# injun-baek/Video-Depth-Normal-v2

Measured on AMD Instinct MI355X. Metric: depth frames/sec at 518x518, ViT-L, higher is better.
Workload: dtype f16x3; 1 GPU; DepthAnythingV2(vitl) batch=8 518x518 streams/GPU, memory bank full (S=6); replicas per GPU; lanes=2, precision=f16x3, ranks=1, backend=none, attention_pv_products=1

## Files before the change

video-depth-normal-v2_amd/csrc/spatial.hip:

```cpp
#include "common.hpp"
#include <stddef.h>

namespace {

__device__ __forceinline__ void ac_coord(int o, float scale, int in, int& i0, int& i1, float& l1) {
#pragma clang fp contract(off)
  const float src = scale * (float)o;
  i0 = (int)src;
  i0 = i0 < in - 1 ? i0 : in - 1;
  i1 = i0 < in - 1 ? i0 + 1 : i0;
  l1 = src - (float)i0;
}

template <int DT>
__global__ __launch_bounds__(256) void upsample_kernel(const typename Half<DT>::T* __restrict__ x,
                                                       const typename Half<DT>::T* __restrict__ xl,
                                                       typename Half<DT>::T* __restrict__ y,
                                                       typename Half<DT>::T* __restrict__ yl, int B, int IH, int IW,
                                                       int OH, int OW, int C) {
  using T = typename Half<DT>::T;
  using V8 = typename Half<DT>::V8;
  const int cv = C >> 3;
  const size_t total = (size_t)B * OH * OW * cv;
  const float sy = OH > 1 ? (float)(IH - 1) / (float)(OH - 1) : 0.f;
  const float sx = OW > 1 ? (float)(IW - 1) / (float)(OW - 1) : 0.f;
  for (size_t i = blockIdx.x * (size_t)256 + threadIdx.x; i < total; i += (size_t)gridDim.x * 256) {
    const int c8 = (int)(i % cv);
    size_t pix = i / cv;
    const int ox = (int)(pix % OW);
    pix /= OW;
    const int oy = (int)(pix % OH);
    const int b = (int)(pix / OH);
    int y0, y1, x0, x1;
    float ly, lx;
    ac_coord(oy, sy, IH, y0, y1, ly);
    ac_coord(ox, sx, IW, x0, x1, lx);
    const size_t xo = (size_t)b * IH * IW * C + c8 * 8;
    const size_t o00 = xo + ((size_t)y0 * IW + x0) * C, o01 = xo + ((size_t)y0 * IW + x1) * C;
    const size_t o10 = xo + ((size_t)y1 * IW + x0) * C, o11 = xo + ((size_t)y1 * IW + x1) * C;
    const V8 v00 = *(const V8*)(x + o00), v01 = *(const V8*)(x + o01);
    const V8 v10 = *(const V8*)(x + o10), v11 = *(const V8*)(x + o11);
    V8 l00, l01, l10, l11, o, ol;
    if (xl) {
      l00 = *(const V8*)(xl + o00); l01 = *(const V8*)(xl + o01);
      l10 = *(const V8*)(xl + o10); l11 = *(const V8*)(xl + o11);
    }
#pragma unroll
    for (int e = 0; e < 8; ++e) {
      float a00 = (float)v00[e], a01 = (float)v01[e], a10 = (float)v10[e], a11 = (float)v11[e];
      if (xl) { a00 += (float)l00[e]; a01 += (float)l01[e]; a10 += (float)l10[e]; a11 += (float)l11[e]; }
      const float top = (1.f - lx) * a00 + lx * a01;
      const float bot = (1.f - lx) * a10 + lx * a11;
      const float r = (1.f - ly) * top + ly * bot;
      if (yl) { T a, b2; split_rtz(r, a, b2); o[e] = a; ol[e] = b2; }
      else o[e] = (T)r;
    }
    *(V8*)(y + i * 8) = o;
    if (yl) *(V8*)(yl + i * 8) = ol;
  }
}

__global__ __launch_bounds__(256) void upsample_f32_kernel(const float* __restrict__ x, float* __restrict__ y, int B,
                                                           int IH, int IW, int OH, int OW, int relu) {
  const size_t total = (size_t)B * OH * OW;
  const float sy = OH > 1 ? (float)(IH - 1) / (float)(OH - 1) : 0.f;
  const float sx = OW > 1 ? (float)(IW - 1) / (float)(OW - 1) : 0.f;
  for (size_t i = blockIdx.x * (size_t)256 + threadIdx.x; i < total; i += (size_t)gridDim.x * 256) {
    const int ox = (int)(i % OW);
    const size_t t = i / OW;
    const int oy = (int)(t % OH);
    const int b = (int)(t / OH);
    int y0, y1, x0, x1;
    float ly, lx;
    ac_coord(oy, sy, IH, y0, y1, ly);
    ac_coord(ox, sx, IW, x0, x1, lx);
    const float* xb = x + (size_t)b * IH * IW;
    const float top = (1.f - lx) * xb[y0 * IW + x0] + lx * xb[y0 * IW + x1];
    const float bot = (1.f - lx) * xb[y1 * IW + x0] + lx * xb[y1 * IW + x1];
    float v = (1.f - ly) * top + ly * bot;
    if (relu) v = fmaxf(v, 0.f);
    y[i] = v;
  }
}

template <int DT>
__global__ __launch_bounds__(256) void patchify_kernel(const float* __restrict__ img,
                                                       typename Half<DT>::T* __restrict__ rows,
                                                       typename Half<DT>::T* __restrict__ rows_lo, int B, int H, int W,
                                                       int ldk) {
  using T = typename Half<DT>::T;
  using V8 = typename Half<DT>::V8;
  const int ph = H / 14, pw = W / 14;
  const int kv = ldk >> 3;
  const size_t total = (size_t)B * ph * pw * kv;
  for (size_t i = blockIdx.x * (size_t)256 + threadIdx.x; i < total; i += (size_t)gridDim.x * 256) {
    const int k8 = (int)(i % kv);
    size_t row = i / kv;
    const int px = (int)(row % pw);
    const size_t t = row / pw;
    const int py = (int)(t % ph);
    const int b = (int)(t / ph);
    V8 o, ol;
#pragma unroll
    for (int e = 0; e < 8; ++e) {
      const int k = k8 * 8 + e;
      float v = 0.f;
      if (k < 588) {
        const int c = k / 196, rem = k - c * 196;
        const int ky = rem / 14, kx = rem - ky * 14;
        v = img[(((size_t)b * 3 + c) * H + py * 14 + ky) * W + px * 14 + kx];
      }
      if (rows_lo) { T a, b2; split_rtz(v, a, b2); o[e] = a; ol[e] = b2; }
      else o[e] = (T)v;
    }
    *(V8*)(rows + i * 8) = o;
    if (rows_lo) *(V8*)(rows_lo + i * 8) = ol;
  }
}

__global__ void fill_row_kernel(float* __restrict__ x, const float* __restrict__ vec, int B, int rows_per_b, int row,
                                int C) {
  const int i = blockIdx.x * blockDim.x + threadIdx.x;
  if (i >= B * C) return;
  const int b = i / C, c = i - b * C;
  x[((size_t)b * rows_per_b + row) * C + c] = vec[c];
}

__device__ __forceinline__ void cubic_w(float t, float w[4]) {
  const float A = -0.75f;
  const float x0 = t + 1.f, x1 = t, x2 = 1.f - t, x3 = 2.f - t;
  w[0] = ((A * x0 - 5.f * A) * x0 + 8.f * A) * x0 - 4.f * A;
  w[1] = ((A + 2.f) * x1 - (A + 3.f)) * x1 * x1 + 1.f;
  w[2] = ((A + 2.f) * x2 - (A + 3.f)) * x2 * x2 + 1.f;
  w[3] = ((A * x3 - 5.f * A) * x3 + 8.f * A) * x3 - 4.f * A;
}

__global__ void bicubic_kernel(const float* __restrict__ src, float* __restrict__ dst, int ih, int iw, int oh, int ow,
                               int C, float inv_sy, float inv_sx) {
  const size_t total = (size_t)oh * ow * C;
  for (size_t i = blockIdx.x * (size_t)blockDim.x + threadIdx.x; i < total; i += (size_t)gridDim.x * blockDim.x) {
    const int c = (int)(i % C);
    const size_t p = i / C;
    const int ox = (int)(p % ow), oy = (int)(p / ow);
    const float fy = ((float)oy + 0.5f) * inv_sy - 0.5f;
    const float fx = ((float)ox + 0.5f) * inv_sx - 0.5f;
    const int iy = (int)floorf(fy), ix = (int)floorf(fx);
    float wy[4], wx[4];
    cubic_w(fy - (float)iy, wy);
    cubic_w(fx - (float)ix, wx);
    float acc = 0.f;
#pragma unroll
    for (int a = 0; a < 4; ++a) {
      int yy = iy - 1 + a;
      yy = yy < 0 ? 0 : (yy > ih - 1 ? ih - 1 : yy);
      float rowv = 0.f;
#pragma unroll
      for (int bq = 0; bq < 4; ++bq) {
        int xx = ix - 1 + bq;
        xx = xx < 0 ? 0 : (xx > iw - 1 ? iw - 1 : xx);
        rowv += wx[bq] * src[((size_t)yy * iw + xx) * C + c];
      }
      acc += wy[a] * rowv;
    }
    dst[i] = acc;
  }
}

__device__ __forceinline__ void halfpixel_coord(int o, int in, int out, int& i, float& t) {
  const long long den = 2ll * out, num = (2ll * o + 1) * in - out;
  long long q = num / den, r = num - q * den;
  if (r < 0) { r += den; --q; }
  i = (int)q;
  t = (float)r / (float)den;
}

struct PrepNorm { float mean[3], inv_std[3]; };
__global__ __launch_bounds__(256) void preprocess_kernel(const uint8_t* __restrict__ src, float* __restrict__ dst, int n, int ih, int iw,
                                                         int oh, int ow, int swap_rb, PrepNorm nm) {
  const size_t per = (size_t)oh * ow, total = per * n;
  for (size_t i = blockIdx.x * (size_t)256 + threadIdx.x; i < total; i += (size_t)gridDim.x * 256) {
    const int f = (int)(i / per);
    const size_t p = i - (size_t)f * per;
    const int ox = (int)(p % ow), oy = (int)(p / ow);
    int iy, ix;
    float ty, tx;
    halfpixel_coord(oy, ih, oh, iy, ty);
    halfpixel_coord(ox, iw, ow, ix, tx);
    float wy[4], wx[4];
    cubic_w(ty, wy);
    cubic_w(tx, wx);
    const uint8_t* img = src + (size_t)f * ih * iw * 3;
    float acc[3] = {0.f, 0.f, 0.f};
#pragma unroll
    for (int a = 0; a < 4; ++a) {
      int yy = iy - 1 + a;
      yy = yy < 0 ? 0 : (yy > ih - 1 ? ih - 1 : yy);
      float rowv[3] = {0.f, 0.f, 0.f};
#pragma unroll
      for (int bq = 0; bq < 4; ++bq) {
        int xx = ix - 1 + bq;
        xx = xx < 0 ? 0 : (xx > iw - 1 ? iw - 1 : xx);
        const uint8_t* px = img + ((size_t)yy * iw + xx) * 3;
#pragma unroll
        for (int c = 0; c < 3; ++c) rowv[c] += wx[bq] * ((float)px[c] / 255.0f);
      }
#pragma unroll
      for (int c = 0; c < 3; ++c) acc[c] += wy[a] * rowv[c];
    }
#pragma unroll
    for (int c = 0; c < 3; ++c) {
      const int sc = swap_rb ? 2 - c : c;
      dst[((size_t)f * 3 + c) * per + p] = (acc[sc] - nm.mean[c]) * nm.inv_std[c];
    }
  }
}

template <int DT>
__global__ __launch_bounds__(256) void head_out_kernel(const typename Half<DT>::T* __restrict__ feat,
                                                       const typename Half<DT>::T* __restrict__ feat_lo,
                                                       const float* __restrict__ w, float bias,
                                                       float* __restrict__ depth, int M, int C, int relu) {
  using V8 = typename Half<DT>::V8;
  __shared__ float sw[64];
  if (threadIdx.x < C) sw[threadIdx.x] = w[threadIdx.x];
  __syncthreads();
  for (size_t m = blockIdx.x * (size_t)256 + threadIdx.x; m < (size_t)M; m += (size_t)gridDim.x * 256) {
    float acc = bias;
    for (int c = 0; c < C; c += 8) {
      const V8 v = *(const V8*)(feat + m * C + c);
#pragma unroll
      for (int e = 0; e < 8; ++e) acc += sw[c + e] * (float)v[e];
      if (feat_lo) {
        const V8 vl = *(const V8*)(feat_lo + m * C + c);
#pragma unroll
        for (int e = 0; e < 8; ++e) acc += sw[c + e] * (float)vl[e];
      }
    }
    depth[m] = relu ? fmaxf(acc, 0.f) : acc;
  }
}

__global__ __launch_bounds__(256) void mask_down1_kernel(const float* __restrict__ depth, float* __restrict__ out,
                                                         int B, int H, int W, int OH, int OW,
                                                         const float* __restrict__ w) {
  __shared__ float sw[53];
  if (threadIdx.x < 53) sw[threadIdx.x] = w[threadIdx.x];
  __syncthreads();
  const size_t total = (size_t)B * OH * OW;
  for (size_t i = blockIdx.x * (size_t)256 + threadIdx.x; i < total; i += (size_t)gridDim.x * 256) {
    const int ox = (int)(i % OW);
    const size_t t = i / OW;
    const int oy = (int)(t % OH);
    const int b = (int)(t / OH);
    float in[9];
#pragma unroll
    for (int ky = 0; ky < 3; ++ky)
#pragma unroll
      for (int kx = 0; kx < 3; ++kx) {
        const int iy = oy * 2 - 1 + ky, ix = ox * 2 - 1 + kx;
        float v = 0.f;
        if (iy >= 0 && iy < H && ix >= 0 && ix < W) v = 1.f / (1.f + expf(-depth[((size_t)b * H + iy) * W + ix]));
        in[ky * 3 + kx] = v;
      }
    float ch[4], mean = 0.f;
#pragma unroll
    for (int c = 0; c < 4; ++c) {
      float a = sw[36 + c];
#pragma unroll
      for (int k = 0; k < 9; ++k) a += sw[c * 9 + k] * in[k];
      ch[c] = a;
      mean += a;
    }
    mean *= 0.25f;
    float var = 0.f;
#pragma unroll
    for (int c = 0; c < 4; ++c) var += (ch[c] - mean) * (ch[c] - mean);
    const float rstd = 1.f / sqrtf(var * 0.25f + 1e-6f);
    float o = sw[52];
#pragma unroll
    for (int c = 0; c < 4; ++c) o += sw[48 + c] * gelu_erf((ch[c] - mean) * rstd * sw[40 + c] + sw[44 + c]);
    out[i] = o;
  }
}

__global__ __launch_bounds__(128) void mask_down2_kernel(const float* __restrict__ in, float* __restrict__ out, int B,
                                                         int H, int W, int OH, int OW, const float* __restrict__ w) {
  __shared__ float sw[2598];
  for (int i = threadIdx.x; i < 2598; i += 128) sw[i] = w[i];
  __syncthreads();
  const size_t i = blockIdx.x * (size_t)128 + threadIdx.x;
  if (i >= (size_t)B * OH * OW) return;
  const int ox = (int)(i % OW);
  const size_t t = i / OW;
  const int oy = (int)(t % OH);
  const int b = (int)(t / OH);
  float px[49];
#pragma unroll
  for (int ky = 0; ky < 7; ++ky)
#pragma unroll
    for (int kx = 0; kx < 7; ++kx) px[ky * 7 + kx] = in[((size_t)b * H + oy * 7 + ky) * W + ox * 7 + kx];
  float ch[49], mean = 0.f;
#pragma unroll
  for (int c = 0; c < 49; ++c) {
    float a = sw[2401 + c];
#pragma unroll
    for (int k = 0; k < 49; ++k) a += sw[c * 49 + k] * px[k];
    ch[c] = a;
    mean += a;
  }
  mean *= (1.f / 49.f);
  float var = 0.f;
#pragma unroll
  for (int c = 0; c < 49; ++c) var += (ch[c] - mean) * (ch[c] - mean);
  const float rstd = 1.f / sqrtf(var * (1.f / 49.f) + 1e-6f);
  float o = sw[2597];
#pragma unroll
  for (int c = 0; c < 49; ++c)
    o += sw[2548 + c] * gelu_erf((ch[c] - mean) * rstd * sw[2450 + c] + sw[2499 + c]);
  out[i] = o;
}

constexpr int DW_TH = 8, DW_CB = 32, DW_PS = 36;
__global__ __launch_bounds__(256) void dwconv7_kernel(const float* __restrict__ x, float* __restrict__ y, int B, int H,
                                                      int W, int C, const float* __restrict__ w,
                                                      const float* __restrict__ bias, int WT) {
  extern __shared__ __attribute__((aligned(16))) char smem[];
  float* sw = (float*)smem;
  float* sx = sw + 49 * DW_CB;
  const int cblocks = C / DW_CB, rtiles = (H + DW_TH - 1) / DW_TH, ctiles = (W + WT - 1) / WT;
  int bid = blockIdx.x;
  const int cb = (bid % cblocks) * DW_CB;
  bid /= cblocks;
  const int x0 = (bid % ctiles) * WT;
  bid /= ctiles;
  const int oy0 = (bid % rtiles) * DW_TH, b = bid / rtiles;
  const int Wt = (W - x0) < WT ? (W - x0) : WT;
  const int WP = WT + 6;
  for (int i = threadIdx.x; i < 49 * (DW_CB / 4); i += 256) {
    const int t = i / (DW_CB / 4), v = i - t * (DW_CB / 4);
    *(f32x4*)(sw + t * DW_CB + v * 4) = *(const f32x4*)(w + (size_t)t * C + cb + v * 4);
  }
  for (int i = threadIdx.x; i < (DW_TH + 6) * WP * (DW_CB / 4); i += 256) {
    const int v = i % (DW_CB / 4);
    const int p = i / (DW_CB / 4);
    const int r = p / WP, cx = p - r * WP;
    const int iy = oy0 - 3 + r, ix = x0 + cx - 3;
    f32x4 val = {0.f, 0.f, 0.f, 0.f};
    if (iy >= 0 && iy < H && ix >= 0 && ix < W) val = *(const f32x4*)(x + (((size_t)b * H + iy) * W + ix) * C + cb + v * 4);
    *(f32x4*)(sx + (size_t)(r * WP + cx) * DW_PS + v * 4) = val;
  }
  __syncthreads();
  const int v = threadIdx.x & 7, pl = threadIdx.x >> 3;
  const int runs_per_row = (Wt + 3) / 4;
  const f32x4 bv = *(const f32x4*)(bias + cb + v * 4);
  for (int run = pl; run < DW_TH * runs_per_row; run += 32) {
    const int ry = run / runs_per_row, ox0 = (run - ry * runs_per_row) * 4;
    if (oy0 + ry >= H) break;
    f32x4 acc[4] = {bv, bv, bv, bv};
#pragma unroll
    for (int ky = 0; ky < 7; ++ky) {
      const float* row = sx + (size_t)((ry + ky) * WP + ox0) * DW_PS + v * 4;
      f32x4 in[10], wk[7];
#pragma unroll
      for (int i = 0; i < 10; ++i) in[i] = (ox0 + i < WP) ? *(const f32x4*)(row + i * DW_PS) : f32x4{0.f, 0.f, 0.f, 0.f};
#pragma unroll
      for (int kx = 0; kx < 7; ++kx) wk[kx] = *(const f32x4*)(sw + (ky * 7 + kx) * DW_CB + v * 4);
#pragma unroll
      for (int o = 0; o < 4; ++o)
#pragma unroll
        for (int kx = 0; kx < 7; ++kx) acc[o] += in[o + kx] * wk[kx];
    }
#pragma unroll
    for (int o = 0; o < 4; ++o)
      if (ox0 + o < Wt) *(f32x4*)(y + (((size_t)b * H + oy0 + ry) * W + x0 + ox0 + o) * C + cb + v * 4) = acc[o];
  }
}

constexpr int OC_T = 16, OC_NT = 512;
__host__ __device__ inline int oc_src0(int o, float scale, int in) {
  const int i0 = (int)(scale * (float)o);
  return i0 < in - 1 ? i0 : in - 1;
}
template <int CS>
__global__ __launch_bounds__(OC_NT) void oc1_combine_kernel(const float* __restrict__ z, const float* __restrict__ bias,
                                                          float* __restrict__ out, int IH, int IW, int OH, int OW, int Co,
                                                          int max_pix) {
  extern __shared__ __attribute__((aligned(16))) char smem[];
  float* sz = (float*)smem;
  constexpr int V = CS / 4;
  const float sy = OH > 1 ? (float)(IH - 1) / (float)(OH - 1) : 0.f;
  const float sx = OW > 1 ? (float)(IW - 1) / (float)(OW - 1) : 0.f;
  const int slices = Co / CS, txn = (OW + OC_T - 1) / OC_T, tyn = (OH + OC_T - 1) / OC_T;
  int bid = blockIdx.x;
  const int cs = (bid % slices) * CS;
  bid /= slices;
  const int ox0 = (bid % txn) * OC_T;
  bid /= txn;
  const int oy0 = (bid % tyn) * OC_T, b = bid / tyn;
  const int ylast = oy0 + OC_T < OH - 1 ? oy0 + OC_T : OH - 1, xlast = ox0 + OC_T < OW - 1 ? ox0 + OC_T : OW - 1;
  const int py0 = oc_src0(oy0 > 0 ? oy0 - 1 : 0, sy, IH), px0 = oc_src0(ox0 > 0 ? ox0 - 1 : 0, sx, IW);
  int py1 = oc_src0(ylast, sy, IH), px1 = oc_src0(xlast, sx, IW);
  py1 = py1 < IH - 1 ? py1 + 1 : py1;
  px1 = px1 < IW - 1 ? px1 + 1 : px1;
  const int nph = py1 - py0 + 1, npw = px1 - px0 + 1;
  if (nph * npw > max_pix) return;
  const float* zb = z + ((size_t)b * IH * IW) * 9 * Co + cs;
  const int total = nph * npw * 9 * V;
  constexpr int U = 9;
  for (int base = threadIdx.x; base < total; base += OC_NT * U) {
    f32x4 r[U];
#pragma unroll
    for (int u = 0; u < U; ++u) {
      const int i = base + u * OC_NT;
      if (i < total) {
        const int v = i % V, t = (i / V) % 9, p = i / (9 * V);
        const int pr = p / npw, pc = p - pr * npw;
        r[u] = *(const f32x4*)(zb + ((size_t)(py0 + pr) * IW + px0 + pc) * 9 * Co + t * Co + v * 4);
      }
    }
#pragma unroll
    for (int u = 0; u < U; ++u) {
      const int i = base + u * OC_NT;
      if (i < total) *(f32x4*)(sz + (size_t)i * 4) = r[u];
    }
  }
  __syncthreads();
  for (int i = threadIdx.x; i < OC_T * OC_T * V; i += OC_NT) {
    const int v = i % V, pix = i / V;
    const int oy = oy0 + pix / OC_T, ox = ox0 + pix % OC_T;
    if (oy >= OH || ox >= OW) continue;
    int xa[3], xb[3];
    float xl[3];
#pragma unroll
    for (int kx = 0; kx < 3; ++kx) {
      const int xx = ox + kx - 1;
      int x0 = 0, x1 = 0;
      float l = 0.f;
      if (xx >= 0 && xx < OW) ac_coord(xx, sx, IW, x0, x1, l);
      xa[kx] = (x0 - px0) * 9 * CS;
      xb[kx] = (x1 - px0) * 9 * CS;
      xl[kx] = l;
    }
    f32x4 acc = *(const f32x4*)(bias + cs + v * 4);
#pragma unroll
    for (int ky = 0; ky < 3; ++ky) {
      const int yy = oy + ky - 1;
      if (yy < 0 || yy >= OH) continue;
      int y0, y1;
      float ly;
      ac_coord(yy, sy, IH, y0, y1, ly);
      const float* r0 = sz + (size_t)(y0 - py0) * npw * 9 * CS + v * 4;
      const float* r1 = sz + (size_t)(y1 - py0) * npw * 9 * CS + v * 4;
#pragma unroll
      for (int kx = 0; kx < 3; ++kx) {
        const int xx = ox + kx - 1;
        if (xx < 0 || xx >= OW) continue;
        const int t = (ky * 3 + kx) * CS;
        const float lx = xl[kx];
        const f32x4 a00 = *(const f32x4*)(r0 + xa[kx] + t), a01 = *(const f32x4*)(r0 + xb[kx] + t);
        const f32x4 a10 = *(const f32x4*)(r1 + xa[kx] + t), a11 = *(const f32x4*)(r1 + xb[kx] + t);
        const float w00 = (1.f - ly) * (1.f - lx), w01 = (1.f - ly) * lx, w10 = ly * (1.f - lx), w11 = ly * lx;
        acc += w00 * a00 + w01 * a01 + (w10 * a10 + w11 * a11);
      }
    }
    *(f32x4*)(out + (((size_t)b * OH + oy) * OW + ox) * Co + cs + v * 4) = acc;
  }
}

inline int grid_for(size_t work, int cap = 4096) {
  const size_t b = (work + 255) / 256;
  return (int)(b < (size_t)cap ? (b ? b : 1) : cap);
}

}

extern "C" int vdn_upsample_bilinear(int dt, const void* x, const void* x_lo, void* y, void* y_lo, int B, int IH,
                                     int IW, int OH, int OW, int C, vdn_stream stream) {
  if (!x || !y || B <= 0 || IH <= 0 || IW <= 0 || OH <= 0 || OW <= 0 || C <= 0) return VDN_EINVAL;
  if ((C & 7) || (((uintptr_t)x | (uintptr_t)y) & 15)) return VDN_EALIGN;
  const int g = grid_for((size_t)B * OH * OW * (C >> 3), 16384);
  hipStream_t s = (hipStream_t)stream;
  return with_half(dt, [&](auto t) -> int {
    using T = typename Half<decltype(t)::value>::T;
    hipLaunchKernelGGL(upsample_kernel<decltype(t)::value>, dim3(g), dim3(256), 0, s, (const T*)x, (const T*)x_lo, (T*)y, (T*)y_lo, B,
                       IH, IW, OH, OW, C);
    VDN_CHECK_LAUNCH();
    return VDN_OK;
  });
}

extern "C" int vdn_upsample_bilinear_f32(const float* x, float* y, int B, int IH, int IW, int OH, int OW, int relu,
                                         vdn_stream stream) {
  if (!x || !y || B <= 0 || IH <= 0 || IW <= 0 || OH <= 0 || OW <= 0) return VDN_EINVAL;
  hipLaunchKernelGGL(upsample_f32_kernel, dim3(grid_for((size_t)B * OH * OW)), dim3(256), 0, (hipStream_t)stream, x, y,
                     B, IH, IW, OH, OW, relu);
  VDN_CHECK_LAUNCH();
  return VDN_OK;
}

extern "C" int vdn_oc1_combine(const float* z, const float* bias, float* out, int B, int IH, int IW, int OH, int OW, int Co,
                               vdn_stream stream) {
  if (!z || !bias || !out || B <= 0 || IH <= 0 || IW <= 0 || OH <= 0 || OW <= 0 || Co <= 0) return VDN_EINVAL;
  if ((Co & 15) || (((uintptr_t)z | (uintptr_t)bias | (uintptr_t)out) & 15)) return VDN_EALIGN;
  const float sy = OH > 1 ? (float)(IH - 1) / (float)(OH - 1) : 0.f;
  const float sx = OW > 1 ? (float)(IW - 1) / (float)(OW - 1) : 0.f;
  auto span = [](int O, int I, float s) {
    int worst = 0;
    for (int o0 = 0; o0 < O; o0 += OC_T) {
      const int last = o0 + OC_T < O - 1 ? o0 + OC_T : O - 1;
      int p1 = oc_src0(last, s, I);
      p1 = p1 < I - 1 ? p1 + 1 : p1;
      const int n = p1 - oc_src0(o0 > 0 ? o0 - 1 : 0, s, I) + 1;
      worst = n > worst ? n : worst;
    }
    return worst;
  };
  const int max_pix = span(OH, IH, sy) * span(OW, IW, sx);
  constexpr int CS = 16;
  const size_t lds = (size_t)max_pix * 9 * CS * sizeof(float);
  if (lds > 160 * 1024) return VDN_EUNSUPPORTED;
  const size_t blocks = (size_t)B * ((OH + OC_T - 1) / OC_T) * ((OW + OC_T - 1) / OC_T) * (Co / CS);
  if (blocks >= (1u << 31)) return VDN_EUNSUPPORTED;
  static const hipError_t attr = hipFuncSetAttribute((const void*)oc1_combine_kernel<CS>, hipFuncAttributeMaxDynamicSharedMemorySize, 160 * 1024);
  if (attr != hipSuccess) return -(1000 + (int)attr);
  hipLaunchKernelGGL(oc1_combine_kernel<CS>, dim3((unsigned)blocks), dim3(OC_NT), lds, (hipStream_t)stream, z, bias, out, IH, IW, OH,
                     OW, Co, max_pix);
  VDN_CHECK_LAUNCH();
  return VDN_OK;
}

extern "C" int vdn_patchify(int dt, const float* img, void* rows, void* rows_lo, int B, int H, int W, int ldk,
                            vdn_stream stream) {
  if (!img || !rows || B <= 0 || H <= 0 || W <= 0 || H % 14 || W % 14) return VDN_EINVAL;
  if (ldk < 588 || (ldk & 63) || ((uintptr_t)rows & 15)) return VDN_EALIGN;
  const int g = grid_for((size_t)B * (H / 14) * (W / 14) * (ldk >> 3), 8192);
  hipStream_t s = (hipStream_t)stream;
  return with_half(dt, [&](auto t) -> int {
    using T = typename Half<decltype(t)::value>::T;
    hipLaunchKernelGGL(patchify_kernel<decltype(t)::value>, dim3(g), dim3(256), 0, s, img, (T*)rows, (T*)rows_lo, B, H, W, ldk);
    VDN_CHECK_LAUNCH();
    return VDN_OK;
  });
}

extern "C" int vdn_fill_row(float* x, const float* vec, int B, int rows_per_b, int row, int C, vdn_stream stream) {
  if (!x || !vec || B <= 0 || rows_per_b <= 0 || row < 0 || row >= rows_per_b || C <= 0) return VDN_EINVAL;
  hipLaunchKernelGGL(fill_row_kernel, dim3((B * C + 255) / 256), dim3(256), 0, (hipStream_t)stream, x, vec, B,
                     rows_per_b, row, C);
  VDN_CHECK_LAUNCH();
  return VDN_OK;
}

extern "C" int vdn_bicubic(const float* src, float* dst, int ih, int iw, int oh, int ow, int C, float scale_rows,
                           float scale_cols, vdn_stream stream) {
  if (!src || !dst || ih <= 0 || iw <= 0 || oh <= 0 || ow <= 0 || C <= 0 || scale_rows <= 0.f || scale_cols <= 0.f)
    return VDN_EINVAL;
  hipLaunchKernelGGL(bicubic_kernel, dim3(grid_for((size_t)oh * ow * C)), dim3(256), 0, (hipStream_t)stream, src, dst,
                     ih, iw, oh, ow, C, 1.0f / scale_rows, 1.0f / scale_cols);
  VDN_CHECK_LAUNCH();
  return VDN_OK;
}

extern "C" int vdn_preprocess(const uint8_t* frames, int n, int h, int w, int swap_rb, float* out, int H, int W, const float* mean3,
                              const float* std3, vdn_stream stream) {
  if (!frames || !out || !mean3 || !std3 || n <= 0 || h <= 0 || w <= 0 || H <= 0 || W <= 0) return VDN_EINVAL;
  PrepNorm nm;
  for (int c = 0; c < 3; ++c) {
    if (!(std3[c] > 0.f)) return VDN_EINVAL;
    nm.mean[c] = mean3[c];
    nm.inv_std[c] = 1.0f / std3[c];
  }
  hipLaunchKernelGGL(preprocess_kernel, dim3(grid_for((size_t)n * H * W)), dim3(256), 0, (hipStream_t)stream, frames, out, n, h, w, H, W,
                     swap_rb, nm);
  VDN_CHECK_LAUNCH();
  return VDN_OK;
}

extern "C" int vdn_head_out(int dt, const void* feat, const void* feat_lo, const float* w, float bias, float* depth,
                            int M, int C, int relu, vdn_stream stream) {
  if (!feat || !w || !depth || M <= 0 || C <= 0 || C > 64) return VDN_EINVAL;
  if ((C & 7) || ((uintptr_t)feat & 15)) return VDN_EALIGN;
  const int g = grid_for((size_t)M, 8192);
  hipStream_t s = (hipStream_t)stream;
  return with_half(dt, [&](auto t) -> int {
    using T = typename Half<decltype(t)::value>::T;
    hipLaunchKernelGGL(head_out_kernel<decltype(t)::value>, dim3(g), dim3(256), 0, s, (const T*)feat, (const T*)feat_lo, w, bias, depth,
                       M, C, relu);
    VDN_CHECK_LAUNCH();
    return VDN_OK;
  });
}

extern "C" int vdn_mask_down1(const float* depth, float* out, int B, int H, int W, int OH, int OW, const float* w,
                              vdn_stream stream) {
  if (!depth || !out || !w || B <= 0 || OH != (H + 2 - 3) / 2 + 1 || OW != (W + 2 - 3) / 2 + 1) return VDN_EINVAL;
  hipLaunchKernelGGL(mask_down1_kernel, dim3(grid_for((size_t)B * OH * OW)), dim3(256), 0, (hipStream_t)stream, depth,
                     out, B, H, W, OH, OW, w);
  VDN_CHECK_LAUNCH();
  return VDN_OK;
}

extern "C" int vdn_mask_down2(const float* in, float* out, int B, int H, int W, int OH, int OW, const float* w,
                              vdn_stream stream) {
  if (!in || !out || !w || B <= 0 || OH != (H - 7) / 7 + 1 || OW != (W - 7) / 7 + 1 || OH <= 0 || OW <= 0)
    return VDN_EINVAL;
  const size_t total = (size_t)B * OH * OW;
  hipLaunchKernelGGL(mask_down2_kernel, dim3((unsigned)((total + 127) / 128)), dim3(128), 0, (hipStream_t)stream, in,
                     out, B, H, W, OH, OW, w);
  VDN_CHECK_LAUNCH();
  return VDN_OK;
}

extern "C" int vdn_dwconv7(const float* x, float* y, int B, int H, int W, int C, const float* w, const float* bias,
                           vdn_stream stream) {
  if (!x || !y || !w || !bias || B <= 0 || H <= 0 || W <= 0 || C <= 0) return VDN_EINVAL;
  if (C % DW_CB) return VDN_EALIGN;
  const int WT = ((size_t)49 * DW_CB + (size_t)(DW_TH + 6) * (W + 6) * DW_PS) * sizeof(float) <= 160 * 1024 ? W : 64;
  const size_t lds = ((size_t)49 * DW_CB + (size_t)(DW_TH + 6) * (WT + 6) * DW_PS) * sizeof(float);
  static const hipError_t attr = hipFuncSetAttribute((const void*)dwconv7_kernel, hipFuncAttributeMaxDynamicSharedMemorySize, 160 * 1024);
  if (attr != hipSuccess) return -(1000 + (int)attr);
  hipLaunchKernelGGL(dwconv7_kernel, dim3(B * ((H + DW_TH - 1) / DW_TH) * ((W + WT - 1) / WT) * (C / DW_CB)), dim3(256), lds,
                     (hipStream_t)stream, x, y, B, H, W, C, w, bias, WT);
  VDN_CHECK_LAUNCH();
  return VDN_OK;
}

extern "C" size_t vdn_sizeof_gemm_desc(void) { return sizeof(vdn_gemm_desc); }
extern "C" size_t vdn_offsetof_gemm_zeros(void) { return offsetof(vdn_gemm_desc, zeros); }
extern "C" size_t vdn_offsetof_gemm_res2_lo(void) { return offsetof(vdn_gemm_desc, res2_lo); }

extern "C" const char* vdn_version(void) { return "vdn-hip 0.1 (gfx950)"; }

extern "C" int vdn_arch_ok(void) {
  hipDeviceProp_t prop;
  if (hipGetDeviceProperties(&prop, 0) != hipSuccess) return 0;
  const char* a = prop.gcnArchName;
  return (a[0] == 'g' && a[1] == 'f' && a[2] == 'x' && a[3] == '9' && a[4] == '5' && a[5] == '0') ? 1 : 0;
}
```

video-depth-normal-v2_amd/csrc/tail.hip:

```cpp
#include "common.hpp"

namespace {

constexpr int TW = 16, TH = 16, PW = TW + 2, PH = TH + 2, NPIX = PW * PH;
constexpr int CB = 32;
constexpr int PWS = 20;
constexpr int PLANE = PH * PWS * 64;
constexpr int SP = 13, SPLANE = SP * SP * 64;
constexpr int SLOADS = (SP * SP * 4 * 2 + 255) / 256;

__device__ __forceinline__ void ac_coord(int o, float scale, int in, int& i0, int& i1, float& l1) {
  const float src = scale * (float)o;
  i0 = (int)src;
  i0 = i0 < in - 1 ? i0 : in - 1;
  i1 = i0 < in - 1 ? i0 + 1 : i0;
  l1 = src - (float)i0;
}

template <int DT>
__global__ __launch_bounds__(256) __attribute__((amdgpu_waves_per_eu(2, 2))) void depth_tail_kernel(const float* __restrict__ x, int B, int IH, int IW,
                                                         int C, const typename Half<DT>::T* __restrict__ w,
                                                         const typename Half<DT>::T* __restrict__ wl, int ldb,
                                                         const float* __restrict__ b2, const float* __restrict__ w1, float b1,
                                                         float* __restrict__ depth, int OH, int OW, int relu) {
  using H = Half<DT>;
  using T = typename H::T;
  using V8 = typename H::V8;
  extern __shared__ __attribute__((aligned(16))) char smem[];
  char* ssrc = smem + 2 * PLANE;

  const int tid = threadIdx.x, lane = tid & 63;
  const int wave = __builtin_amdgcn_readfirstlane(tid >> 6);
  const int tiles_x = (OW + TW - 1) / TW, tiles_y = (OH + TH - 1) / TH;
  const int tile = xcd_remap(blockIdx.x, gridDim.x);
  const int b = tile / (tiles_x * tiles_y);
  const int trem = tile - b * tiles_x * tiles_y;
  const int ty0 = (trem / tiles_x) * TH, tx0 = (trem % tiles_x) * TW;
  const float sy = OH > 1 ? (float)(IH - 1) / (float)(OH - 1) : 0.f;
  const float sx = OW > 1 ? (float)(IW - 1) / (float)(OW - 1) : 0.f;
  const float* xb = x + (size_t)b * IH * IW * C;

  const int fr = lane & 15, fq = lane >> 4;
  const int wj = wave & 1, wr = wave >> 1;
  f32x4 acc[8];
#pragma unroll
  for (int i = 0; i < 8; ++i) acc[i] = f32x4{0.f, 0.f, 0.f, 0.f};
  const T* wrow = w + (size_t)(16 * wj + fr) * ldb + fq * 8;
  const ptrdiff_t wdelta = (const char*)wl - (const char*)w;
  u32x4 wh[9], wlo[9];
  const char* abase[3][4];
#pragma unroll
  for (int kx = 0; kx < 3; ++kx)
#pragma unroll
    for (int rm = 0; rm < 4; ++rm)
      abase[kx][rm] = smem + (wr * 8 * PWS + fr + kx) * 64 + ((fq ^ ((rm + ((fr + kx) >> 2)) & 3)) << 4);

  int dummy;
  float dl;
  int sy0, sx0;
  ac_coord(ty0 > 0 ? ty0 - 1 : 0, sy, IH, sy0, dummy, dl);
  ac_coord(tx0 > 0 ? tx0 - 1 : 0, sx, IW, sx0, dummy, dl);
  auto dma_src = [&](int cb) {
    int tid_d = tid;
    asm volatile("" : "+v"(tid_d));
#pragma unroll
    for (int i = 0; i < SLOADS; ++i) {
      const int it = tid_d + i * 256;
      if (it < SP * SP * 8) {
        const int pix = it >> 3, c4 = it & 7;
        int yy = sy0 + pix / SP, xx = sx0 + pix % SP;
        yy = yy < IH ? yy : IH - 1;
        xx = xx < IW ? xx : IW - 1;
        const float* src = xb + ((size_t)yy * IW + xx) * C + cb + c4 * 4;
        __builtin_amdgcn_global_load_lds((const __attribute__((address_space(1))) void*)src,
                                         (__attribute__((address_space(3))) void*)(ssrc + (i * 4 + wave) * 1024), 16, 0, 0);
      }
    }
  };
  dma_src(0);
  asm volatile("s_waitcnt vmcnt(0)" ::: "memory");

  for (int cb = 0; cb < C; cb += CB) {
    __syncthreads();
#pragma unroll
    for (int tap = 0; tap < 9; ++tap) {
      wh[tap] = *(const u32x4*)(wrow + tap * C + cb);
      wlo[tap] = *(const u32x4*)((const char*)(wrow + tap * C + cb) + wdelta);
    }
    int tid_c = tid;
    asm volatile("" : "+v"(tid_c));
    for (int it = tid_c; it < NPIX * 4; it += 256) {
      const int pix = it >> 2, ch = it & 3;
      const int py = pix / PW, px = pix - py * PW;
      const int gy = ty0 - 1 + py, gx = tx0 - 1 + px;
      V8 oh, ol;
#pragma unroll
      for (int e = 0; e < 8; ++e) { oh[e] = (T)0.f; ol[e] = (T)0.f; }
      if (gy >= 0 && gy < OH && gx >= 0 && gx < OW) {
        int y0, y1, x0, x1;
        float ly, lx;
        ac_coord(gy, sy, IH, y0, y1, ly);
        ac_coord(gx, sx, IW, x0, x1, lx);
        const float* c00 = (const float*)ssrc + ((y0 - sy0) * SP + (x0 - sx0)) * 32 + ch * 8;
        const float* c01 = (const float*)ssrc + ((y0 - sy0) * SP + (x1 - sx0)) * 32 + ch * 8;
        const float* c10 = (const float*)ssrc + ((y1 - sy0) * SP + (x0 - sx0)) * 32 + ch * 8;
        const float* c11 = (const float*)ssrc + ((y1 - sy0) * SP + (x1 - sx0)) * 32 + ch * 8;
        f32x4 a00[2], a01[2], a10[2], a11[2];
#pragma unroll
        for (int u = 0; u < 2; ++u) {
          a00[u] = *(const f32x4*)(c00 + 4 * u); a01[u] = *(const f32x4*)(c01 + 4 * u);
          a10[u] = *(const f32x4*)(c10 + 4 * u); a11[u] = *(const f32x4*)(c11 + 4 * u);
        }
#pragma unroll
        for (int e = 0; e < 8; e += 2) {
          float r[2];
#pragma unroll
          for (int q = 0; q < 2; ++q) {
            const int u = (e + q) >> 2, k = (e + q) & 3;
            const float top = (1.f - lx) * a00[u][k] + lx * a01[u][k];
            const float bot = (1.f - lx) * a10[u][k] + lx * a11[u][k];
            r[q] = (1.f - ly) * top + ly * bot;
          }
          T h0, h1, q0, q1;
          split2_rtz(r[0], r[1], h0, h1, q0, q1);
          oh[e] = h0; oh[e + 1] = h1; ol[e] = q0; ol[e + 1] = q1;
        }
      }
      const int off = (py * PWS + px) * 64 + ((ch ^ ((py + (px >> 2)) & 3)) << 4);
      *(V8*)(smem + off) = oh;
      *(V8*)(smem + PLANE + off) = ol;
    }
    asm volatile("s_waitcnt vmcnt(0)"
                 : "+v"(wh[0]), "+v"(wh[1]), "+v"(wh[2]), "+v"(wh[3]), "+v"(wh[4]), "+v"(wh[5]), "+v"(wh[6]), "+v"(wh[7]), "+v"(wh[8]),
                   "+v"(wlo[0]), "+v"(wlo[1]), "+v"(wlo[2]), "+v"(wlo[3]), "+v"(wlo[4]), "+v"(wlo[5]), "+v"(wlo[6]), "+v"(wlo[7]),
                   "+v"(wlo[8])
                 :
                 : "memory");
    __syncthreads();
    if (cb + CB < C) dma_src(cb + CB);
    {
      V8 fh[2], fl[2];
      auto rd = [&](int idx, V8& h, V8& l) {
        const int kx = idx / 10, rho = idx - kx * 10;
        const char* ap = abase[kx][rho & 3] + rho * (PWS * 64);
        h = *(const V8*)ap;
        l = *(const V8*)(ap + PLANE);
      };
      rd(0, fh[0], fl[0]);
#pragma unroll
      for (int idx = 0; idx < 30; ++idx) {
        const int kx = idx / 10, rho = idx - kx * 10, cur = idx & 1;
        if (idx + 1 < 30) rd(idx + 1, fh[cur ^ 1], fl[cur ^ 1]);
#pragma unroll
        for (int ky = 0; ky < 3; ++ky) {
          const int i = rho - ky, tap = ky * 3 + kx;
          if (i >= 0 && i < 8) {
            f32x4 c = acc[i];
            c = H::mfma16(__builtin_bit_cast(V8, wh[tap]), fl[cur], c);
            c = H::mfma16(__builtin_bit_cast(V8, wlo[tap]), fh[cur], c);
            c = H::mfma16(__builtin_bit_cast(V8, wh[tap]), fh[cur], c);
            acc[i] = c;
          }
        }
      }
    }
    asm volatile("s_waitcnt vmcnt(0)" ::: "memory");
  }

  const f32x4 bias4 = *(const f32x4*)(b2 + wj * 16 + fq * 4), w14 = *(const f32x4*)(w1 + wj * 16 + fq * 4);
  __syncthreads();
  float* part = (float*)smem;
#pragma unroll
  for (int i = 0; i < 8; ++i) {
    float sum = 0.f;
#pragma unroll
    for (int e = 0; e < 4; ++e) {
      float v = acc[i][e] + bias4[e];
      v = (v < 0.f) ? 0.f : v;
      sum = fmaf(v, w14[e], sum);
    }
    sum += __shfl_xor(sum, 16);
    sum += __shfl_xor(sum, 32);
    if (fq == 0) part[wj * (TH * TW) + (wr * 8 + i) * TW + fr] = sum;
  }
  __syncthreads();
  {
    const int py = tid >> 4, px = tid & 15;
    float v = part[py * TW + px] + part[TH * TW + py * TW + px] + b1;
    if (relu) v = (v < 0.f) ? 0.f : v;
    const int oy = ty0 + py, ox = tx0 + px;
    if (oy < OH && ox < OW) depth[((size_t)b * OH + oy) * OW + ox] = v;
  }
}

}

extern "C" int vdn_depth_tail(int dt, const float* x, int B, int IH, int IW, int C, const void* w,
                              const void* w_lo, int ldb, const float* bias2, const float* w1, float b1, float* depth, int OH,
                              int OW, int relu, vdn_stream stream) {
  if (!x || !w || !w_lo || !bias2 || !w1 || !depth || B <= 0 || IH <= 0 || IW <= 0 || OH <= 0 || OW <= 0) return VDN_EINVAL;
  if (C <= 0 || (C % CB) || ldb < 9 * C || (ldb & 7)) return VDN_EALIGN;
  const float sy = OH > 1 ? (float)(IH - 1) / (float)(OH - 1) : 0.f, sx = OW > 1 ? (float)(IW - 1) / (float)(OW - 1) : 0.f;
  if ((int)(17.f * sy) + 3 > SP || (int)(17.f * sx) + 3 > SP) return VDN_EUNSUPPORTED;
  if (((uintptr_t)x | (uintptr_t)w | (uintptr_t)w_lo | (uintptr_t)bias2 | (uintptr_t)w1) & 15) return VDN_EALIGN;
  const int tiles = B * ((OH + TH - 1) / TH) * ((OW + TW - 1) / TW);
  hipStream_t s = (hipStream_t)stream;
  return with_half(dt, [&](auto t) -> int {
    using T = typename Half<decltype(t)::value>::T;
    hipLaunchKernelGGL(depth_tail_kernel<decltype(t)::value>, dim3(tiles), dim3(256), 2 * PLANE + 2 * SPLANE, s, x, B, IH, IW, C,
                       (const T*)w, (const T*)w_lo, ldb, bias2, w1, b1, depth, OH, OW, relu);
    VDN_CHECK_LAUNCH();
    return VDN_OK;
  });
}
```

Measured before the change: 287.2 frames/s.

## Separate oc1 combine into staged horizontal/vertical passes and strip-tile depth tail

Adds a new oc1 combine kernel that first interpolates horizontally and sums the kx taps into LDS per source row, then interpolates vertically. Each block now covers a 16-wide output strip and can take 32-channel slices. This cuts redundant LDS staging and global reads of the 9-tap z tensor. The depth tail kernel now processes strips of S=3 horizontal tiles per block, reusing the conv weight registers loaded once per channel block across tiles. The cost is three times the accumulator registers, which raises spill and occupancy risk under the waves_per_eu(2,2) constraint.

Result: no change. 288.5 frames/s (median of 6 runs) (+0.5%).

```diff
diff --git a/video-depth-normal-v2_amd/csrc/spatial.hip b/video-depth-normal-v2_amd/csrc/spatial.hip
--- a/video-depth-normal-v2_amd/csrc/spatial.hip
+++ b/video-depth-normal-v2_amd/csrc/spatial.hip
@@ -467,6 +467,88 @@
   }
 }
 
+constexpr int OC2_TX = 16;
+template <int CS>
+__global__ __launch_bounds__(OC_NT) void oc1_combine2_kernel(const float* __restrict__ z, const float* __restrict__ bias,
+                                                           float* __restrict__ out, int IH, int IW, int OH, int OW, int Co,
+                                                           int max_rows) {
+  extern __shared__ __attribute__((aligned(16))) char smem[];
+  float* sh = (float*)smem;
+  constexpr int V = CS / 4, TX = OC2_TX;
+  const float sy = OH > 1 ? (float)(IH - 1) / (float)(OH - 1) : 0.f;
+  const float sx = OW > 1 ? (float)(IW - 1) / (float)(OW - 1) : 0.f;
+  const int slices = Co / CS, txn = (OW + TX - 1) / TX, tyn = (OH + OC_T - 1) / OC_T;
+  int bid = xcd_remap(blockIdx.x, gridDim.x);
+  const int ox0 = (bid % txn) * TX;
+  bid /= txn;
+  const int oy0 = (bid % tyn) * OC_T;
+  bid /= tyn;
+  const int cs = (bid % slices) * CS, b = bid / slices;
+  const int ylast = oy0 + OC_T < OH - 1 ? oy0 + OC_T : OH - 1;
+  const int py0 = oc_src0(oy0 > 0 ? oy0 - 1 : 0, sy, IH);
+  int py1 = oc_src0(ylast, sy, IH);
+  py1 = py1 < IH - 1 ? py1 + 1 : py1;
+  const int nph = py1 - py0 + 1;
+  if (nph > max_rows) return;
+  const float* zb = z + ((size_t)b * IH * IW) * 9 * Co + cs;
+  const int total = 3 * nph * TX * V;
+  for (int i = threadIdx.x; i < total; i += OC_NT) {
+    const int v = i % V, col = (i / V) % TX, rk = i / (V * TX);
+    const int ky = rk / nph, r = rk - ky * nph;
+    const int ox = ox0 + col < OW ? ox0 + col : OW - 1;
+    const float* zr = zb + ((size_t)(py0 + r) * IW) * 9 * Co + ky * 3 * Co + v * 4;
+    f32x4 a[3][2];
+    float l[3];
+    bool ok[3];
+#pragma unroll
+    for (int kx = 0; kx < 3; ++kx) {
+      const int xx = ox + kx - 1;
+      ok[kx] = xx >= 0 && xx < OW;
+      int x0, x1;
+      ac_coord(ok[kx] ? xx : ox, sx, IW, x0, x1, l[kx]);
+      a[kx][0] = *(const f32x4*)(zr + (size_t)x0 * 9 * Co + kx * Co);
+      a[kx][1] = *(const f32x4*)(zr + (size_t)x1 * 9 * Co + kx * Co);
+    }
+    f32x4 h = {0.f, 0.f, 0.f, 0.f};
+#pragma unroll
+    for (int kx = 0; kx < 3; ++kx)
+      if (ok[kx]) h += (1.f - l[kx]) * a[kx][0] + l[kx] * a[kx][1];
+    *(f32x4*)(sh + (size_t)i * 4) = h;
+  }
+  __syncthreads();
+  for (int i = threadIdx.x; i < OC_T * TX * V; i += OC_NT) {
+    const int v = i % V, pix = i / V;
+    const int col = pix % TX, oy = oy0 + pix / TX, ox = ox0 + col;
+    if (oy >= OH || ox >= OW) continue;
+    f32x4 acc = *(const f32x4*)(bias + cs + v * 4);
+    const float* hc = sh + col * CS + v * 4;
+#pragma unroll
+    for (int ky = 0; ky < 3; ++ky) {
+      const int yy = oy + ky - 1;
+      if (yy < 0 || yy >= OH) continue;
+      int y0, y1;
+      float ly;
+      ac_coord(yy, sy, IH, y0, y1, ly);
+      const f32x4 h0 = *(const f32x4*)(hc + (size_t)(ky * nph + y0 - py0) * TX * CS);
+      const f32x4 h1 = *(const f32x4*)(hc + (size_t)(ky * nph + y1 - py0) * TX * CS);
+      acc += (1.f - ly) * h0 + ly * h1;
+    }
+    *(f32x4*)(out + (((size_t)b * OH + oy) * OW + ox) * Co + cs + v * 4) = acc;
+  }
+}
+
+template <int CS>
+int launch_oc1_combine2(const float* z, const float* bias, float* out, int B, int IH, int IW, int OH, int OW, int Co, int rows,
+                        size_t lds, hipStream_t s) {
+  const size_t blocks = (size_t)B * ((OH + OC_T - 1) / OC_T) * ((OW + OC2_TX - 1) / OC2_TX) * (Co / CS);
+  if (blocks >= (1u << 31)) return VDN_EUNSUPPORTED;
+  static const hipError_t attr = hipFuncSetAttribute((const void*)oc1_combine2_kernel<CS>, hipFuncAttributeMaxDynamicSharedMemorySize, 160 * 1024);
+  if (attr != hipSuccess) return -(1000 + (int)attr);
+  hipLaunchKernelGGL(oc1_combine2_kernel<CS>, dim3((unsigned)blocks), dim3(OC_NT), lds, s, z, bias, out, IH, IW, OH, OW, Co, rows);
+  VDN_CHECK_LAUNCH();
+  return VDN_OK;
+}
+
 inline int grid_for(size_t work, int cap = 4096) {
   const size_t b = (work + 255) / 256;
   return (int)(b < (size_t)cap ? (b ? b : 1) : cap);
@@ -515,10 +597,16 @@
     }
     return worst;
   };
-  const int max_pix = span(OH, IH, sy) * span(OW, IW, sx);
+  const int rows = span(OH, IH, sy), max_pix = rows * span(OW, IW, sx);
   constexpr int CS = 16;
   const size_t lds = (size_t)max_pix * 9 * CS * sizeof(float);
   if (lds > 160 * 1024) return VDN_EUNSUPPORTED;
+  const char* v1 = getenv("VDN_OC1_COMBINE_V1");
+  const size_t lds2 = (size_t)3 * rows * OC2_TX * CS * sizeof(float);
+  if (!(v1 && v1[0] == '1') && lds2 <= 160 * 1024) {
+    if (!(Co & 31) && 2 * lds2 <= 80 * 1024) return launch_oc1_combine2<32>(z, bias, out, B, IH, IW, OH, OW, Co, rows, 2 * lds2, (hipStream_t)stream);
+    return launch_oc1_combine2<CS>(z, bias, out, B, IH, IW, OH, OW, Co, rows, lds2, (hipStream_t)stream);
+  }
   const size_t blocks = (size_t)B * ((OH + OC_T - 1) / OC_T) * ((OW + OC_T - 1) / OC_T) * (Co / CS);
   if (blocks >= (1u << 31)) return VDN_EUNSUPPORTED;
   static const hipError_t attr = hipFuncSetAttribute((const void*)oc1_combine_kernel<CS>, hipFuncAttributeMaxDynamicSharedMemorySize, 160 * 1024);
diff --git a/video-depth-normal-v2_amd/csrc/tail.hip b/video-depth-normal-v2_amd/csrc/tail.hip
--- a/video-depth-normal-v2_amd/csrc/tail.hip
+++ b/video-depth-normal-v2_amd/csrc/tail.hip
@@ -17,7 +17,7 @@
   l1 = src - (float)i0;
 }
 
-template <int DT>
+template <int DT, int S>
 __global__ __launch_bounds__(256) __attribute__((amdgpu_waves_per_eu(2, 2))) void depth_tail_kernel(const float* __restrict__ x, int B, int IH, int IW,
                                                          int C, const typename Half<DT>::T* __restrict__ w,
                                                          const typename Half<DT>::T* __restrict__ wl, int ldb,
@@ -32,19 +32,24 @@
   const int tid = threadIdx.x, lane = tid & 63;
   const int wave = __builtin_amdgcn_readfirstlane(tid >> 6);
   const int tiles_x = (OW + TW - 1) / TW, tiles_y = (OH + TH - 1) / TH;
-  const int tile = xcd_remap(blockIdx.x, gridDim.x);
-  const int b = tile / (tiles_x * tiles_y);
-  const int trem = tile - b * tiles_x * tiles_y;
-  const int ty0 = (trem / tiles_x) * TH, tx0 = (trem % tiles_x) * TW;
+  const int strips_x = (tiles_x + S - 1) / S;
+  const int strip = xcd_remap(blockIdx.x, gridDim.x);
+  const int b = strip / (strips_x * tiles_y);
+  const int srem = strip - b * strips_x * tiles_y;
+  const int sxi = srem % strips_x;
+  const int ty0 = (srem / strips_x) * TH, txs = sxi * S * TW;
+  const int nt = tiles_x - sxi * S < S ? tiles_x - sxi * S : S;
   const float sy = OH > 1 ? (float)(IH - 1) / (float)(OH - 1) : 0.f;
   const float sx = OW > 1 ? (float)(IW - 1) / (float)(OW - 1) : 0.f;
   const float* xb = x + (size_t)b * IH * IW * C;
 
   const int fr = lane & 15, fq = lane >> 4;
   const int wj = wave & 1, wr = wave >> 1;
-  f32x4 acc[8];
-#pragma unroll
-  for (int i = 0; i < 8; ++i) acc[i] = f32x4{0.f, 0.f, 0.f, 0.f};
+  f32x4 acc[S][8];
+#pragma unroll
+  for (int s = 0; s < S; ++s)
+#pragma unroll
+    for (int i = 0; i < 8; ++i) acc[s][i] = f32x4{0.f, 0.f, 0.f, 0.f};
   const T* wrow = w + (size_t)(16 * wj + fr) * ldb + fq * 8;
   const ptrdiff_t wdelta = (const char*)wl - (const char*)w;
   u32x4 wh[9], wlo[9];
@@ -57,10 +62,16 @@
 
   int dummy;
   float dl;
-  int sy0, sx0;
+  int sy0;
   ac_coord(ty0 > 0 ? ty0 - 1 : 0, sy, IH, sy0, dummy, dl);
-  ac_coord(tx0 > 0 ? tx0 - 1 : 0, sx, IW, sx0, dummy, dl);
-  auto dma_src = [&](int cb) {
+  auto src_x0 = [&](int tx0) {
+    int x0, d1;
+    float d2;
+    ac_coord(tx0 > 0 ? tx0 - 1 : 0, sx, IW, x0, d1, d2);
+    return x0;
+  };
+  auto dma_src = [&](int cb, int tx0) {
+    const int sx0 = src_x0(tx0);
     int tid_d = tid;
     asm volatile("" : "+v"(tid_d));
 #pragma unroll
@@ -77,15 +88,22 @@
       }
     }
   };
-  dma_src(0);
+  dma_src(0, txs);
   asm volatile("s_waitcnt vmcnt(0)" ::: "memory");
 
   for (int cb = 0; cb < C; cb += CB) {
-    __syncthreads();
-#pragma unroll
-    for (int tap = 0; tap < 9; ++tap) {
-      wh[tap] = *(const u32x4*)(wrow + tap * C + cb);
-      wlo[tap] = *(const u32x4*)((const char*)(wrow + tap * C + cb) + wdelta);
+#pragma unroll
+   for (int s = 0; s < S; ++s) {
+    if (s > 0 && s >= nt) continue;
+    const int tx0 = txs + s * TW;
+    const int sx0 = src_x0(tx0);
+    __syncthreads();
+    if (s == 0) {
+#pragma unroll
+      for (int tap = 0; tap < 9; ++tap) {
+        wh[tap] = *(const u32x4*)(wrow + tap * C + cb);
+        wlo[tap] = *(const u32x4*)((const char*)(wrow + tap * C + cb) + wdelta);
+      }
     }
     int tid_c = tid;
     asm volatile("" : "+v"(tid_c));
@@ -130,6 +148,7 @@
       *(V8*)(smem + off) = oh;
       *(V8*)(smem + PLANE + off) = ol;
     }
+    if (s == 0)
     asm volatile("s_waitcnt vmcnt(0)"
                  : "+v"(wh[0]), "+v"(wh[1]), "+v"(wh[2]), "+v"(wh[3]), "+v"(wh[4]), "+v"(wh[5]), "+v"(wh[6]), "+v"(wh[7]), "+v"(wh[8]),
                    "+v"(wlo[0]), "+v"(wlo[1]), "+v"(wlo[2]), "+v"(wlo[3]), "+v"(wlo[4]), "+v"(wlo[5]), "+v"(wlo[6]), "+v"(wlo[7]),
@@ -137,7 +156,8 @@
                  :
                  : "memory");
     __syncthreads();
-    if (cb + CB < C) dma_src(cb + CB);
+    if (s + 1 < S && s + 1 < nt) dma_src(cb, tx0 + TW);
+    else if (cb + CB < C) dma_src(cb + CB, txs);
     {
       V8 fh[2], fl[2];
       auto rd = [&](int idx, V8& h, V8& l) {
@@ -155,42 +175,64 @@
         for (int ky = 0; ky < 3; ++ky) {
           const int i = rho - ky, tap = ky * 3 + kx;
           if (i >= 0 && i < 8) {
-            f32x4 c = acc[i];
+            f32x4 c = acc[s][i];
             c = H::mfma16(__builtin_bit_cast(V8, wh[tap]), fl[cur], c);
             c = H::mfma16(__builtin_bit_cast(V8, wlo[tap]), fh[cur], c);
             c = H::mfma16(__builtin_bit_cast(V8, wh[tap]), fh[cur], c);
-            acc[i] = c;
+            acc[s][i] = c;
           }
         }
       }
     }
     asm volatile("s_waitcnt vmcnt(0)" ::: "memory");
+   }
   }
 
   const f32x4 bias4 = *(const f32x4*)(b2 + wj * 16 + fq * 4), w14 = *(const f32x4*)(w1 + wj * 16 + fq * 4);
-  __syncthreads();
   float* part = (float*)smem;
 #pragma unroll
-  for (int i = 0; i < 8; ++i) {
-    float sum = 0.f;
-#pragma unroll
-    for (int e = 0; e < 4; ++e) {
-      float v = acc[i][e] + bias4[e];
-      v = (v < 0.f) ? 0.f : v;
-      sum = fmaf(v, w14[e], sum);
-    }
-    sum += __shfl_xor(sum, 16);
-    sum += __shfl_xor(sum, 32);
-    if (fq == 0) part[wj * (TH * TW) + (wr * 8 + i) * TW + fr] = sum;
+  for (int s = 0; s < S; ++s) {
+    if (s > 0 && s >= nt) continue;
+    __syncthreads();
+#pragma unroll
+    for (int i = 0; i < 8; ++i) {
+      float sum = 0.f;
+#pragma unroll
+      for (int e = 0; e < 4; ++e) {
+        float v = acc[s][i][e] + bias4[e];
+        v = (v < 0.f) ? 0.f : v;
+        sum = fmaf(v, w14[e], sum);
+      }
+      sum += __shfl_xor(sum, 16);
+      sum += __shfl_xor(sum, 32);
+      if (fq == 0) part[wj * (TH * TW) + (wr * 8 + i) * TW + fr] = sum;
+    }
+    __syncthreads();
+    {
+      const int py = tid >> 4, px = tid & 15;
+      float v = part[py * TW + px] + part[TH * TW + py * TW + px] + b1;
+      if (relu) v = (v < 0.f) ? 0.f : v;
+      const int oy = ty0 + py, ox = txs + s * TW + px;
+      if (oy < OH && ox < OW) depth[((size_t)b * OH + oy) * OW + ox] = v;
+    }
   }
-  __syncthreads();
-  {
-    const int py = tid >> 4, px = tid & 15;
-    float v = part[py * TW + px] + part[TH * TW + py * TW + px] + b1;
-    if (relu) v = (v < 0.f) ? 0.f : v;
-    const int oy = ty0 + py, ox = tx0 + px;
-    if (oy < OH && ox < OW) depth[((size_t)b * OH + oy) * OW + ox] = v;
-  }
+}
+
+constexpr int TAIL_STRIP = 3;
+inline int tail_strip() {
+  const char* e = getenv("VDN_TAIL_STRIP");
+  const int s = e ? atoi(e) : 0;
+  return s >= 1 && s <= 4 ? s : TAIL_STRIP;
+}
+
+template <int DT, int S>
+void launch_tail(hipStream_t s, const float* x, int B, int IH, int IW, int C, const void* w, const void* wl, int ldb,
+                 const float* b2, const float* w1, float b1, float* depth, int OH, int OW, int relu) {
+  using T = typename Half<DT>::T;
+  const int tiles_x = (OW + TW - 1) / TW;
+  const int strips = B * ((OH + TH - 1) / TH) * ((tiles_x + S - 1) / S);
+  hipLaunchKernelGGL((depth_tail_kernel<DT, S>), dim3(strips), dim3(256), 2 * PLANE + 2 * SPLANE, s, x, B, IH, IW, C, (const T*)w,
+                     (const T*)wl, ldb, b2, w1, b1, depth, OH, OW, relu);
 }
 
 }
@@ -203,12 +245,16 @@
   const float sy = OH > 1 ? (float)(IH - 1) / (float)(OH - 1) : 0.f, sx = OW > 1 ? (float)(IW - 1) / (float)(OW - 1) : 0.f;
   if ((int)(17.f * sy) + 3 > SP || (int)(17.f * sx) + 3 > SP) return VDN_EUNSUPPORTED;
   if (((uintptr_t)x | (uintptr_t)w | (uintptr_t)w_lo | (uintptr_t)bias2 | (uintptr_t)w1) & 15) return VDN_EALIGN;
-  const int tiles = B * ((OH + TH - 1) / TH) * ((OW + TW - 1) / TW);
   hipStream_t s = (hipStream_t)stream;
+  const int strip = tail_strip();
   return with_half(dt, [&](auto t) -> int {
-    using T = typename Half<decltype(t)::value>::T;
-    hipLaunchKernelGGL(depth_tail_kernel<decltype(t)::value>, dim3(tiles), dim3(256), 2 * PLANE + 2 * SPLANE, s, x, B, IH, IW, C,
-                       (const T*)w, (const T*)w_lo, ldb, bias2, w1, b1, depth, OH, OW, relu);
+    constexpr int DT = decltype(t)::value;
+    switch (strip) {
+      case 1: launch_tail<DT, 1>(s, x, B, IH, IW, C, w, w_lo, ldb, bias2, w1, b1, depth, OH, OW, relu); break;
+      case 2: launch_tail<DT, 2>(s, x, B, IH, IW, C, w, w_lo, ldb, bias2, w1, b1, depth, OH, OW, relu); break;
+      case 3: launch_tail<DT, 3>(s, x, B, IH, IW, C, w, w_lo, ldb, bias2, w1, b1, depth, OH, OW, relu); break;
+      default: launch_tail<DT, 4>(s, x, B, IH, IW, C, w, w_lo, ldb, bias2, w1, b1, depth, OH, OW, relu); break;
+    }
     VDN_CHECK_LAUNCH();
     return VDN_OK;
   });
```
